# hahnec/stofnet

Hardware: AMD Instinct MI355X
Metric: RF waveforms/sec StofNet inference rf_scale=10 (higher is better)
Workload: dtype f32 via split-fp16 x3 MFMA operands (hi+lo, fp32 accumulate), device-side exact-f32 re-run on fp16 range overflow; 1 GPU; C2 StofNet.forward [4096,1,2000] -> [4096,1,20000] per GPU, upsample_factor=10, SemiGlobalBlock on, seeded-random weights (seed 3008); rows_per_gpu=4096, L=2000, upsample_factor=10, precision=auto

## Files before the change

stofnet_amd/build.py:

```python
from __future__ import annotations

import os
import shutil
import subprocess
import sys

HERE = os.path.dirname(os.path.abspath(__file__))
CSRC = os.path.join(HERE, 'csrc')
LIB = os.path.join(HERE, 'libstofnet_amd.so')
SOURCES = ['pack_weights.cpp', 'convstack.hip', 'shuffle_picker.hip', 'hilbert.hip', 'gradpeak.hip', 'gradpeak_f64.hip', 'neighbors.hip', 'train.hip', 'zonzini.hip', 'sincnet.hip', 'riders.hip']
ARCH = 'gfx950'
EXTRA_FLAGS = {'convstack.hip': ['-fno-slp-vectorize']}


def _hipcc() -> str:
    for cand in (os.environ.get('HIPCC'), shutil.which('hipcc'), '/opt/rocm/bin/hipcc'):
        if cand and os.path.exists(cand):
            return cand
    raise RuntimeError('hipcc not found: the HIP extension cannot be built')


def needs_build() -> bool:
    if not os.path.exists(LIB):
        return True
    t = os.path.getmtime(LIB)
    deps = [os.path.join(CSRC, f) for f in os.listdir(CSRC) if f.endswith(('.hip', '.cpp', '.h'))] + [os.path.join(HERE, '..', 'include', 'stofnet_amd.h')]
    return any(os.path.getmtime(d) > t for d in deps)


def build(force: bool = False, verbose: bool = True) -> str:
    if not force and not needs_build():
        return LIB
    hipcc = _hipcc()
    objdir = os.path.join(HERE, 'build')
    os.makedirs(objdir, exist_ok=True)
    objs = []
    procs = []
    for src in SOURCES:
        path = os.path.join(CSRC, src)
        if not os.path.exists(path):
            raise RuntimeError(f'listed source {path} is missing: refusing to link a library without its symbols')
        obj = os.path.join(objdir, os.path.splitext(src)[0] + '.o')
        cmd = [hipcc, '-O3', '-std=c++17', '-fPIC', '-fconstexpr-steps=100000000', f'--offload-arch={ARCH}', '-x', 'hip'] + \
              EXTRA_FLAGS.get(src, []) + ['-c', path, '-o', obj]
        if verbose:
            print(' '.join(cmd), flush=True)
        procs.append((src, subprocess.Popen(cmd, stdout=subprocess.PIPE, stderr=subprocess.STDOUT, text=True)))
        objs.append(obj)
    for src, pr in procs:
        out, _ = pr.communicate()
        if pr.returncode != 0:
            raise RuntimeError(f'hipcc failed on {src}:\n{out}')
        if verbose and out.strip():
            print(out)
    cmd = [hipcc, '-shared', '-fPIC', f'--offload-arch={ARCH}', '-o', LIB] + objs
    if verbose:
        print(' '.join(cmd), flush=True)
    subprocess.run(cmd, check=True)
    return LIB


if __name__ == '__main__':
    build(force='--force' in sys.argv)
    print(LIB)
```

stofnet_amd/csrc/convstack.hip:

```cpp
#include <hip/hip_runtime.h>
#include <stdlib.h>
#include <type_traits>
#include "stof_common.h"
#include "stof_hip_util.h"

namespace stof {
int launch_conv_cl(const float* x, const float* w, const float* bias, const float* residual, const float* saved, float* y,
                   int64_t N, int64_t L, int32_t cin, int32_t cout, int32_t K, int32_t act, int32_t precision,
                   int32_t period, int32_t valid_len, hipStream_t stream, const int* run_if);
}

using namespace stof;

typedef float floatx16 __attribute__((ext_vector_type(16)));
typedef _Float16 half8 __attribute__((ext_vector_type(8)));
typedef _Float16 half4 __attribute__((ext_vector_type(4)));

namespace {

constexpr int LAG_LAST = 34;
constexpr int SGB_NW = 2;
constexpr int SGB_WAVES_PER_SIMD = (SGB_NW <= 2) ? 2 : 1;
constexpr int ROWB = ROWF * 4;

typedef float float2v __attribute__((ext_vector_type(2)));
typedef float floatx4 __attribute__((ext_vector_type(4)));
typedef _Float16 half2v __attribute__((ext_vector_type(2)));

__device__ __forceinline__ int layer_lag(int j) { return j <= 11 ? 3 * j : LAG_LAST; }

__device__ __forceinline__ float4 ld4(const float* p) { return *reinterpret_cast<const float4*>(p); }
__device__ __forceinline__ void st4(float* p, float4 v) { *reinterpret_cast<float4*>(p) = v; }
__device__ __forceinline__ uint4 ldq(const char* p) { return *reinterpret_cast<const uint4*>(p); }

__device__ __forceinline__ float4 as_f4(uint4 v) {
    return make_float4(__uint_as_float(v.x), __uint_as_float(v.y), __uint_as_float(v.z), __uint_as_float(v.w));
}
__device__ __forceinline__ half8 as_h8(uint4 v) {
    union { uint4 u; half8 h; } c;
    c.u = v;
    return c.h;
}

__device__ __forceinline__ floatx16 mma_fp32(uint4 a, uint4 b, floatx16 c) {
    const float4 af = as_f4(a), bf = as_f4(b);
    c = __builtin_amdgcn_mfma_f32_32x32x2f32(af.x, bf.x, c, 0, 0, 0);
    c = __builtin_amdgcn_mfma_f32_32x32x2f32(af.y, bf.y, c, 0, 0, 0);
    c = __builtin_amdgcn_mfma_f32_32x32x2f32(af.z, bf.z, c, 0, 0, 0);
    c = __builtin_amdgcn_mfma_f32_32x32x2f32(af.w, bf.w, c, 0, 0, 0);
    return c;
}

__device__ __forceinline__ int act_frag_off(int frag, int hh, int lh) { return (32 * hh + 8 * frag + 4 * lh) * 4; }

template <int PREC>
__device__ __forceinline__ void store_act4(char* row, int c0, float4 v) {
    if constexpr (PREC == STOF_PREC_FP32) {
        *reinterpret_cast<float4*>(row + 4 * c0) = v;
    } else {
        half4 hi, lo;
        hi[0] = (_Float16)v.x; hi[1] = (_Float16)v.y; hi[2] = (_Float16)v.z; hi[3] = (_Float16)v.w;
        lo[0] = (_Float16)(v.x - (float)hi[0]); lo[1] = (_Float16)(v.y - (float)hi[1]);
        lo[2] = (_Float16)(v.z - (float)hi[2]); lo[3] = (_Float16)(v.w - (float)hi[3]);
        *reinterpret_cast<half4*>(row + 2 * c0) = hi;
        *reinterpret_cast<half4*>(row + 128 + 2 * c0) = lo;
    }
}

__device__ __forceinline__ float opaque_one() {
    float one;
    asm volatile("s_mov_b32 %0, 1.0" : "=s"(one));
    return one;
}
__device__ __forceinline__ float mix_add(_Float16 h, float v, float one) { return __builtin_fmaf((float)h, one, v); }
__device__ __forceinline__ float mix_sub(_Float16 h, float v, float one) { return __builtin_fmaf(-(float)h, one, v); }
__device__ __forceinline__ half2v cvt_h2(float a, float b) {
    const float2v v = {a, b};
    return __builtin_convertvector(v, half2v);
}
__device__ __forceinline__ unsigned h2_bits(half2v h) {
    union { half2v h; unsigned u; } c;
    c.h = h;
    return c.u;
}
__device__ __forceinline__ half2v bits_h2(unsigned u) {
    union { half2v h; unsigned u; } c;
    c.u = u;
    return c.h;
}
// ... 800 lines not shown
                    for (int gg = 0; gg < 4; ++gg) epi_store(NT - 1, gg, o[gg]);
                };
                if (inplace) tail(std::true_type{});
                else tail(std::false_type{});
                STAMP_ADD(5);
                __syncthreads();
                STAMP_ADD(2);
                continue;
            }
            auto last_chunks = [&]() {
#pragma unroll
                for (int cc = 0; cc < BODY_CHUNKS_LAST; cc += 2) { do_chunk(wf[0], bf0, bf1, cc); do_chunk(wf[1], bf1, bf0, cc + 1); }
            };
            last_chunks();
            STAMP_ADD(4);

            {
                bool valid[NT];
                int tt[NT], nn[NT];
#pragma unroll
                for (int k = 0; k < NT; ++k) {
                    const int off = 32 * (NT * ni + k) + ln;
                    const int g = R0 + off;
                    decode_row(nR, tR, off, nn[k], tt[k]);
                    int nw, tw;
                    vmap(n0 + nn[k], tt[k], nw, tw);
                    valid[k] = (g >= 0) && (g < gend) && (tt[k] < L) && (tw >= 0) && (tw < Ltrue) &&
                               (tt[k] >= p.halo) && (tt[k] < p.halo + p.seg_len);
                    nn[k] = nw - n0;
                    tt[k] = tw;
                }
                if (p.status != nullptr) {
                    bool bad = false;
#pragma unroll
                    for (int k = 0; k < NT; ++k)
#pragma unroll
                        for (int e = 0; e < 16; ++e) bad = bad || !(fabsf(acc[k][e]) <= 3.0e38f);
                    if (__any(bad) && lane == 0) atomicOr(p.status, 1);
                }
#pragma unroll
                for (int k = 0; k < NT; ++k) {
                    if (!valid[k]) continue;
                    float* const orow = p.y + ((size_t)(n0 + nn[k]) * Ltrue + tt[k]) * r;
#pragma unroll
                    for (int gg = 0; gg < 4; ++gg) {
                        const int c0 = 32 * mi + 8 * gg + 4 * lh;
                        if (c0 >= r) continue;
                        const float vv[4] = {acc[k][4 * gg], acc[k][4 * gg + 1], acc[k][4 * gg + 2], acc[k][4 * gg + 3]};
                        if ((r & 3) == 0) {
                            st4(orow + c0, make_float4(vv[0], vv[1], vv[2], vv[3]));
                        } else {
#pragma unroll
                            for (int e = 0; e < 4; ++e)
                                if (c0 + e < r) orow[c0 + e] = vv[e];
                        }
                    }
                }
            }
            STAMP_ADD(5);
            __syncthreads();
            STAMP_ADD(2);
            }
        }
    }
#ifdef STOF_STAMPS
    if (lane == 0 && p.stamps) {
        unsigned long long* o = p.stamps + ((size_t)blockIdx.x * 4 + wave) * 8;
        for (int i = 0; i < 6; ++i) o[i] = tsum[i];
        o[6] = stamp() - tstart;
        o[7] = (unsigned long long)nsteps;
    }
#endif
}

constexpr int BODY_P2_C1F = 640;
#include "body_p2.h"

struct SgbParams {
    const float* x;
    float* pooled;
    const float* c1;
    const float* cbias;
    const float* chunks;
    int N, L, P, tiles_per_wf;
    const int* run_if;
    unsigned char* arg;
};

template <int PREC, int NW, bool ARG = false>
__global__ __launch_bounds__(256, SGB_WAVES_PER_SIMD) void sgb_contract_pool_kernel(const SgbParams p) {
    constexpr int SHAPE = PREC == STOF_PREC_F16X3 ? 16 : 32;
    static_assert(!ARG || PREC == STOF_PREC_F16X3, "the arg-max output lives in the split-fp16 form");
    static_assert(NW % 2 == 0, "80*NW must be a multiple of 32");
    constexpr int ROWS = SGB_SCALE * NW;
    constexpr int MT = ROWS / 32;
    constexpr int TR = ROWS + 4;
    constexpr int RAWN = TR + 8;
    constexpr int RF = SHAPE == 16 ? ROWF16 : ROWF;
    constexpr int ROWB = RF * 4;
    extern __shared__ __attribute__((aligned(16))) float smem[];
    char* const act = reinterpret_cast<char*>(smem);
    float* const raw = smem + TR * RF;

    const int tid = threadIdx.x;
    const int lane = tid & 63, wave = tid >> 6;
    const int ln = lane & 31, lh = lane >> 5;
    const int n = blockIdx.x / p.tiles_per_wf;
    const int w0 = (blockIdx.x - n * p.tiles_per_wf) * NW;
    const int L = p.L;
    const int tbase = SGB_SCALE * w0 - 2;
    if (p.run_if != nullptr && *p.run_if == 0) return;

    const uint4* const wbase = reinterpret_cast<const uint4*>(p.chunks) + wave * 64 + lane;
    auto wload = [&](int c, int f) -> uint4 { return wbase[((size_t)c * FRAGS_PER_CHUNK + f) * 256]; };
    uint4 wf[2][FRAGS_PER_CHUNK];
#pragma unroll
    for (int f = 0; f < FRAGS_PER_CHUNK; ++f) {
        wf[0][f] = wload(0, f);
        wf[1][f] = wload(1, f);
    }

    for (int i = tid; i < RAWN; i += 256) {
        const int t = tbase - 4 + i;
        raw[i] = (t >= 0 && t < L) ? p.x[(size_t)n * L + t] : 0.f;
    }
    __syncthreads();
    {
        const int cq = tid & 15, rl = tid >> 4;
        float w1[4][9], b1[4];
#pragma unroll
        for (int i = 0; i < 4; ++i) {
#pragma unroll
            for (int d = 0; d < 9; ++d) w1[i][d] = p.c1[(4 * cq + i) * 10 + d];
            b1[i] = p.c1[(4 * cq + i) * 10 + 9];
        }
        for (int row = rl; row < TR; row += 16) {
            const int t = tbase + row;
            float v[4];
#pragma unroll
            for (int i = 0; i < 4; ++i) {
                float a = b1[i];
#pragma unroll
                for (int d = 0; d < 9; ++d) a = fmaf(w1[i][d], raw[row + d], a);
                v[i] = fmaxf(a, 0.f);
            }
            const bool valid = (t >= 0) && (t < L);
            store_act4<PREC>(act + row * ROWB, 4 * cq,
                             valid ? make_float4(v[0], v[1], v[2], v[3]) : make_float4(0.f, 0.f, 0.f, 0.f));
        }
    }
    __syncthreads();

    int c = 0;
    if constexpr (SHAPE == 16) {
        constexpr int MW = SGB_SCALE / 16;
        const int j16 = lane & 15, q4 = lane >> 4;
        for (int ocb = 0; ocb < 4; ++ocb) {
            floatx4 acc[NW][MW][2];
#pragma unroll
            for (int w = 0; w < NW; ++w)
#pragma unroll
                for (int m = 0; m < MW; ++m)
#pragma unroll
                    for (int nt = 0; nt < 2; ++nt)
#pragma unroll
                        for (int e = 0; e < 4; ++e) acc[w][m][nt][e] = 0.f;
            constexpr int NUNIT = 10 * NW;
            auto aload = [&](uint4 (&a)[MW][2], int uu) {
                const int cc = uu / NW, w = uu % NW;
                const int d = cc >> 1, hh = cc & 1;
                const char* arow = act + (SGB_SCALE * w + j16 + d) * ROWB + 64 * hh + 16 * q4;
#pragma unroll
                for (int m = 0; m < MW; ++m) {
                    a[m][0] = ldq(arow + 16 * m * ROWB);
                    a[m][1] = ldq(arow + 16 * m * ROWB + 128);
                }
            };
            auto mfma16 = [](const uint4& a, const uint4& b, floatx4 cacc) {
                return __builtin_amdgcn_mfma_f32_16x16x32_f16(as_h8(a), as_h8(b), cacc, 0, 0, 0);
            };
            auto do_unit = [&](uint4 (&acur)[MW][2], uint4 (&anext)[MW][2], int uu) {
                const int cc = uu / NW, w = uu % NW;
                uint4 (&wq)[FRAGS_PER_CHUNK] = wf[cc & 1];
                const int c2 = (c + 2 < SGB_NCHUNK) ? c + 2 : 0;
                aload(anext, uu + 1 < NUNIT ? uu + 1 : 0);
#pragma unroll
                for (int m = 0; m < MW; ++m) {
                    acc[w][m][0] = mfma16(acur[m][0], wq[0], acc[w][m][0]);
                    acc[w][m][1] = mfma16(acur[m][0], wq[2], acc[w][m][1]);
                    acc[w][m][0] = mfma16(acur[m][1], wq[0], acc[w][m][0]);
                    acc[w][m][1] = mfma16(acur[m][1], wq[2], acc[w][m][1]);
                    acc[w][m][0] = mfma16(acur[m][0], wq[1], acc[w][m][0]);
                    acc[w][m][1] = mfma16(acur[m][0], wq[3], acc[w][m][1]);
                }
                if (w == NW - 1) {
#pragma unroll
                    for (int f = 0; f < FRAGS_PER_CHUNK; ++f) wq[f] = wload(c2, f);
                    ++c;
                }
#pragma unroll
                for (int i = 0; i < MW * 2; ++i) {
                    __builtin_amdgcn_sched_group_barrier(0x008, 3, 0);
                    __builtin_amdgcn_sched_group_barrier(0x100, 1, 0);
                }
                if (w == NW - 1) __builtin_amdgcn_sched_group_barrier(0x020, FRAGS_PER_CHUNK, 0);
                __builtin_amdgcn_sched_barrier(0);
            };
            uint4 af0[MW][2], af1[MW][2];
            if (ocb == 0) aload(af0, 0);
            static_assert(NUNIT % 2 == 0, "units alternate between two fragment sets");
#pragma unroll
            for (int uu = 0; uu < NUNIT; uu += 2) {
                do_unit(af0, af1, uu);
                do_unit(af1, af0, uu + 1);
            }
#pragma unroll
            for (int nt = 0; nt < 2; ++nt) {
                const int oc = 128 * ocb + 32 * wave + 16 * nt + j16;
                const float bias = p.cbias[oc];
#pragma unroll
                for (int w = 0; w < NW; ++w) {
                    float mval = -INFINITY;
                    if constexpr (ARG) {
                        int bi = 0;
#pragma unroll
                        for (int m = 0; m < MW; ++m)
#pragma unroll
                            for (int e = 0; e < 4; ++e) {
                                const float v = acc[w][m][nt][e];
                                const bool up = v > mval;
                                mval = up ? v : mval;
                                bi = up ? 16 * m + 4 * q4 + e : bi;
                            }
#pragma unroll
                        for (int off = 16; off <= 32; off <<= 1) {
                            const float ov = __shfl_xor(mval, off);
                            const int oi = __shfl_xor(bi, off);
                            const bool take = (ov > mval) || (ov == mval && oi < bi);
                            mval = take ? ov : mval;
                            bi = take ? oi : bi;
                        }
                        if (q4 == 0 && w0 + w < p.P) p.arg[((size_t)n * p.P + w0 + w) * NF_SGB + oc] = (unsigned char)bi;
                    } else {
#pragma unroll
                        for (int m = 0; m < MW; ++m)
#pragma unroll
                            for (int e = 0; e < 4; ++e) mval = fmaxf(mval, acc[w][m][nt][e]);
                        mval = fmaxf(mval, __shfl_xor(mval, 16));
                        mval = fmaxf(mval, __shfl_xor(mval, 32));
                    }
                    mval += bias;
                    mval = mval > 0.f ? mval : 0.01f * mval;
                    if (q4 == 0 && w0 + w < p.P)
                        p.pooled[((size_t)n * p.P + w0 + w) * NF_SGB + oc] = mval;
                }
            }
        }
    } else {
    for (int ocb = 0; ocb < 4; ++ocb) {
        floatx16 acc[MT];
#pragma unroll
        for (int m = 0; m < MT; ++m)
#pragma unroll
            for (int e = 0; e < 16; ++e) acc[m][e] = 0.f;

        constexpr int UPC = FRAGS_PER_CHUNK;
        constexpr int NUNIT = 10 * UPC;
        auto aload = [&](uint4 (&a)[MT], int uu) {
            const int cc = uu / UPC, sub = uu % UPC;
            const int d = cc >> 1, hh = cc & 1;
            const char* arow = act + (ln + d) * ROWB;
#pragma unroll
            for (int m = 0; m < MT; ++m) a[m] = ldq(arow + 32 * m * ROWB + act_frag_off(sub, hh, lh));
        };
        auto do_unit = [&](uint4 (&acur)[MT], uint4 (&anext)[MT], int uu) {
            const int cc = uu / UPC, sub = uu % UPC;
            uint4 (&w)[FRAGS_PER_CHUNK] = wf[cc & 1];
            const int c2 = (c + 2 < SGB_NCHUNK) ? c + 2 : 0;
            aload(anext, uu + 1 < NUNIT ? uu + 1 : 0);
#pragma unroll
            for (int m = 0; m < MT; ++m) acc[m] = mma_fp32(acur[m], w[sub], acc[m]);
            w[sub] = wload(c2, sub);
#pragma unroll
            for (int i = 0; i < MT; ++i) {
                __builtin_amdgcn_sched_group_barrier(0x008, 4, 0);
                __builtin_amdgcn_sched_group_barrier(0x100, 1, 0);
            }
            if (sub == UPC - 1) ++c;
            __builtin_amdgcn_sched_barrier(0);
        };
        uint4 af0[MT], af1[MT];
        if (ocb == 0) aload(af0, 0);
#pragma unroll
        for (int uu = 0; uu < NUNIT; uu += 2) {
            do_unit(af0, af1, uu);
            do_unit(af1, af0, uu + 1);
        }
        const int oc = 128 * ocb + 32 * wave + ln;
        const float bias = p.cbias[oc];
        float wmax[NW];
#pragma unroll
        for (int w = 0; w < NW; ++w) wmax[w] = -INFINITY;
#pragma unroll
        for (int m = 0; m < MT; ++m)
#pragma unroll
            for (int v = 0; v < 16; ++v) {
                const int w = (32 * m + 8 * (v >> 2)) / SGB_SCALE;
                wmax[w] = fmaxf(wmax[w], acc[m][v]);
            }
#pragma unroll
        for (int w = 0; w < NW; ++w) {
            float mval = fmaxf(wmax[w], __shfl_xor(wmax[w], 32));
            mval += bias;
            mval = mval > 0.f ? mval : 0.01f * mval;
            if (lh == 0 && w0 + w < p.P)
                p.pooled[((size_t)n * p.P + w0 + w) * NF_SGB + oc] = mval;
        }
    }
    }
}

__global__ __launch_bounds__(256) void onsets_finalize_kernel(const OnsetPartial* __restrict__ ws, int nslots, int nb, int r,
                                                              int half, int* __restrict__ counts, int* __restrict__ idx,
                                                              long long idx_cap) {
    const int lane = threadIdx.x & 63;
    const int row = blockIdx.x * 4 + (threadIdx.x >> 6);
    if (row >= nb) return;
    const OnsetPartial* e = ws + (size_t)row * nslots;
    float m = -INFINITY, lo = INFINITY;
    for (int s = lane; s < nslots; s += 64)
        if (e[s].written) { m = fmaxf(m, e[s].m); lo = fminf(lo, e[s].lo); }
#pragma unroll
    for (int o = 32; o > 0; o >>= 1) { m = fmaxf(m, __shfl_xor(m, o)); lo = fminf(lo, __shfl_xor(lo, o)); }
    const bool emit = (m > 0.f) || (m < 0.f && (lo == m || half == 0));
    int nout = 0;
    if (emit) {
        const unsigned long long lt_mask = (lane == 0) ? 0ull : (~0ull >> (64 - lane));
        int* out = idx + (long long)row * idx_cap;
        for (int s0 = 0; s0 < nslots; s0 += 64) {
            const int sl = s0 + lane;
            unsigned long long match = __ballot(sl < nslots && e[sl].written && e[sl].m == m);
            while (match) {
            const int s = s0 + __builtin_ctzll(match);
            match &= match - 1;
            const OnsetPartial p = e[s];
            for (int q0 = 0; q0 < 16 * r; q0 += 64) {
                const int q = q0 + lane, j = q / r, c = q - j * r;
                const bool hit = q < 16 * r && ((p.eq[c & 3] >> (j + 16 * (c >> 2))) & 1ull);
                const unsigned long long hm = __ballot(hit);
                if (hit) {
                    const long long pos = nout + __builtin_popcountll(hm & lt_mask);
                    if (pos < idx_cap) out[pos] = (p.tw_base + j) * r + c;
                }
                nout += __builtin_popcountll(hm);
            }
            }
        }
    }
    if (lane == 0) counts[row] = nout;
}

constexpr int BODY_S = 192, BODY_RING = 256, BODY_RAWRING = 256;
inline bool body_p2_rows_ok(int seg_len, int halo) { return seg_len + 2 * halo + GAP >= 2 * BODY_S; }
constexpr int ONSET_MAX_SEGS = 32;

constexpr int64_t onset_seg_slots(int64_t seg_len) { return seg_len / 16 + 2; }
constexpr int64_t onset_max_slots(int64_t L) { return L / 16 + 3 * ONSET_MAX_SEGS; }

struct OnsetArgs {
    OnsetPartial* ws;
    int32_t* counts;
    int32_t* idx;
    int64_t idx_cap;
    int half;
};
constexpr int64_t SUB_BATCH = 4096;

constexpr size_t sgb_lds_bytes(int rowf) {
    return (size_t)((SGB_SCALE * SGB_NW + 4) * rowf + SGB_SCALE * SGB_NW + 12) * sizeof(float);
}

template <int PREC>
int launch_forward(const stof_net_desc* desc, const void* packed_dev, const float* x, float* y, int64_t N,
                   int64_t L, void* workspace, hipStream_t stream, void* const* events, int32_t* status,
                   const int32_t* run_if, const OnsetArgs* onsets = nullptr) {
    const int force_nseg_log2 = desc->seg_policy > 0 ? desc->seg_policy - 1 : -1;
    const int r = desc->upsample_factor;
    const bool has_sgb = desc->semi_global_scale != 1;
    const int64_t P = L / SGB_SCALE;
    const int64_t rem = L - P * SGB_SCALE;

    const float* base = static_cast<const float*>(packed_dev);
    uint64_t off = sizeof(PackedHeader) / sizeof(float);
    const float* c1 = base + off;      off += 64 * 10;
    const float* bias = base + off;    off += 13 * 64;
    const float* body = base + off;    off += (uint64_t)BODY_NCHUNK * BODY_CHUNK_F;
    const float* last16 = nullptr;
    if (PREC == STOF_PREC_F16X3 && r <= 16) { last16 = base + off; off += LAST16_F; }
    const float* cbias = base + off;   off += NF_SGB;
    const float* cchunks = base + off; off += (uint64_t)SGB_NCHUNK * SGB_CHUNK_F;
    const float* ew = base + off;      off += 5ull * NF_SGB * NF;
    const float* ebias = base + off;

    static const bool body_p2 = PREC == STOF_PREC_F16X3 && body_p2_enabled();
    constexpr int RF = PREC == STOF_PREC_F16X3 ? ROWF16 : ROWF;
    using Lds = BodyLds<BODY_S, BODY_RING, BODY_RAWRING, RF>;
    const size_t body_p2_bytes = Lds::BYTES + BODY_P2_C1F * sizeof(float);
    const auto body_kernel = &body_sweep_kernel<PREC, BODY_S, BODY_RING, BODY_RAWRING>;
    const auto body_p2_kernel = &body_sweep_p2_kernel<BODY_S, BODY_RING, BODY_RAWRING>;
    const auto sgb_kernel = &sgb_contract_pool_kernel<PREC, SGB_NW>;
    const size_t sgb_bytes = sgb_lds_bytes(RF);
    static LdsLimitOnce body_lds, body_p2_lds, sgb_lds;
    if (int st = body_lds.ensure(reinterpret_cast<const void*>(body_kernel), (int)Lds::BYTES)) return st;
    if (body_p2)
        if (int st = body_p2_lds.ensure(reinterpret_cast<const void*>(body_p2_kernel), (int)body_p2_bytes)) return st;
    if (int st = sgb_lds.ensure(reinterpret_cast<const void*>(sgb_kernel), (int)sgb_bytes)) return st;
    const int ncu = device_cu_count();

    for (int64_t b0 = 0; b0 < N; b0 += SUB_BATCH) {
        const int64_t nb = (N - b0) < SUB_BATCH ? (N - b0) : SUB_BATCH;
        const float* xb = x + b0 * L;
        float* yb = y ? y + b0 * L * r : nullptr;
        float* pooled = nullptr;
        float* sgb = nullptr;
        const bool ev = events && b0 == 0;
        if (ev) (void)hipEventRecord(static_cast<hipEvent_t>(events[0]), stream);
        if (has_sgb && P > 0) {
            pooled = static_cast<float*>(workspace);
            sgb = pooled + nb * P * NF_SGB;
            SgbParams sp;
            sp.x = xb; sp.pooled = pooled; sp.c1 = c1; sp.cbias = cbias; sp.chunks = cchunks;
            sp.N = (int)nb; sp.L = (int)L; sp.P = (int)P;
            sp.tiles_per_wf = (int)((P + SGB_NW - 1) / SGB_NW);
            sp.run_if = run_if;
            sp.arg = nullptr;
            hipLaunchKernelGGL(sgb_kernel, dim3((unsigned)(nb * sp.tiles_per_wf)), dim3(256), sgb_bytes, stream, sp);
            if (ev) (void)hipEventRecord(static_cast<hipEvent_t>(events[1]), stream);
            {
                const int st = stof::launch_conv_cl(pooled, ew, ebias, nullptr, nullptr, sgb, 1, nb * (P + 2), NF_SGB, NF, 5,
                                                     2, PREC, (int)(P + 2), (int)P, stream, run_if);
                if (st != STOF_OK) return st;
            }
            if (ev) (void)hipEventRecord(static_cast<hipEvent_t>(events[2]), stream);
        } else if (ev) {
            (void)hipEventRecord(static_cast<hipEvent_t>(events[1]), stream);
            (void)hipEventRecord(static_cast<hipEvent_t>(events[2]), stream);
        }
        BodyParams bp;
        bp.x = xb; bp.sgb = (has_sgb && P > 0) ? sgb : nullptr; bp.y = yb;
        bp.c1 = c1; bp.bias = bias; bp.chunks = body; bp.last16 = last16;
        bp.N = (int)nb; bp.L = (int)L; bp.r = r; bp.P = (int)P; bp.rem_half = (int)(rem / 2);
        bp.stamps = nullptr;
        bp.dump = nullptr; bp.dump_stride = 0;
        bp.gin = nullptr; bp.fwd_dump = nullptr;
        bp.status = status;
        bp.run_if = run_if;
        bp.nseg_log2 = 0;
        {
            int64_t best = -1;
            for (int k = 0; k <= 5; ++k) {
                const int64_t ns = (int64_t)1 << k;
                if (k > 0 && L / ns < BODY_S / 2) break;
                const int64_t lv = (L + ns - 1) / ns + (k > 0 ? 76 : 0);
                const int64_t nvk = nb * ns;
                const int64_t w = nvk < ncu ? nvk : ncu;
                const int64_t per = (nvk + w - 1) / w;
                const int64_t steps = (per * (lv + GAP) - GAP + LAG_LAST + BODY_S - 1) / BODY_S;
                if (best < 0 || steps < best) { best = steps; bp.nseg_log2 = k; }
            }
        }
        int64_t nseg = (int64_t)1 << bp.nseg_log2;
        if (force_nseg_log2 >= 0) { bp.nseg_log2 = force_nseg_log2; nseg = (int64_t)1 << force_nseg_log2; }
        bp.seg_len = (int)((L + nseg - 1) / nseg);
        bp.halo = nseg > 1 ? 38 : 0;
        const int64_t nv = nb * nseg;
        bp.N = (int)nv;
        bp.onset_ws = nullptr; bp.onset_slots = 0; bp.onset_seg_slots = 0;
        if (onsets != nullptr) {
            bp.onset_seg_slots = (int)onset_seg_slots(bp.seg_len);
            bp.onset_slots = (int)(nseg * bp.onset_seg_slots);
            bp.onset_ws = onsets->ws;
            if (hipMemsetAsync(onsets->ws, 0, (size_t)nb * bp.onset_slots * sizeof(OnsetPartial), stream) != hipSuccess)
                return STOF_ERR_HIP;
        }
#ifdef STOF_STAMPS
        if (workspace) bp.stamps = reinterpret_cast<unsigned long long*>(static_cast<char*>(workspace) + (size_t)(nb * P * (NF_SGB + NF)) * sizeof(float) + 256);
#endif
        int64_t wgs = nv < ncu ? nv : ncu;
        bp.wf_per_wg = (int)((nv + wgs - 1) / wgs);
        wgs = (nv + bp.wf_per_wg - 1) / bp.wf_per_wg;
        if (body_p2 && body_p2_rows_ok(bp.seg_len, bp.halo))
            hipLaunchKernelGGL(body_p2_kernel, dim3((unsigned)wgs), dim3(256), body_p2_bytes, stream, bp);
        else
            hipLaunchKernelGGL(body_kernel, dim3((unsigned)wgs), dim3(256), Lds::BYTES, stream, bp);
        if (ev) (void)hipEventRecord(static_cast<hipEvent_t>(events[3]), stream);
        if (onsets != nullptr)
            hipLaunchKernelGGL(onsets_finalize_kernel, dim3((unsigned)((nb + 3) / 4)), dim3(256), 0, stream, onsets->ws,
                               bp.onset_slots, (int)nb, r, onsets->half, onsets->counts + b0, onsets->idx + b0 * onsets->idx_cap,
                               (long long)onsets->idx_cap);
    }
    if (hipGetLastError() != hipSuccess) return STOF_ERR_HIP;
    return STOF_OK;
}

int forward_impl(const stof_net_desc* desc, const void* packed_dev, const float* x, float* y, int64_t N, int64_t L,
                 void* workspace, size_t workspace_bytes, void* stream_, void* const* events, int32_t* status,
                 const int32_t* run_if = nullptr, const OnsetArgs* onsets = nullptr) {
    if (!desc || N < 0 || L < 0) return STOF_ERR_BAD_ARG;
    if (desc->precision != STOF_PREC_FP32 && desc->precision != STOF_PREC_F16X3) return STOF_ERR_UNSUPPORTED;
    if (desc->seg_policy < 0 || desc->seg_policy > 6) return STOF_ERR_UNSUPPORTED;
    const int r = desc->upsample_factor;
    if (r < 1 || r > 64) return STOF_ERR_UNSUPPORTED;
    const bool has_sgb = desc->semi_global_scale != 1;
    if (has_sgb && desc->semi_global_scale != SGB_SCALE) return STOF_ERR_UNSUPPORTED;
    const int64_t P = L / SGB_SCALE;
    if (has_sgb && L > 0 && P == 0) return STOF_ERR_POOL_EMPTY;
    if (has_sgb && ((L - P * SGB_SCALE) & 1)) return STOF_ERR_ODD_SGB_REMAINDER;
    if (N == 0 || L == 0) return STOF_OK;
    if (!packed_dev || !x || (!y && !onsets)) return STOF_ERR_BAD_ARG;
    if ((L + GAP) * SUB_BATCH > 0x7fffffffLL) return STOF_ERR_UNSUPPORTED;
    if (has_sgb && (!workspace || workspace_bytes < stof_forward_workspace_bytes(desc, N, L)))
        return STOF_ERR_WORKSPACE;
    hipStream_t stream = static_cast<hipStream_t>(stream_);
// ... 230 lines not shown
    bp.x = x; bp.sgb = has_sgb ? sgb_expand : nullptr; bp.y = y;
    bp.c1 = base; bp.bias = base + 640; bp.chunks = base + 640 + 13 * 64;
    bp.last16 = r <= 16 ? bp.chunks + (size_t)BODY_NCHUNK * BODY_CHUNK_F : nullptr;
    bp.L = (int)L; bp.r = r; bp.P = (int)P; bp.rem_half = (int)((L - P * SGB_SCALE) / 2);
    bp.stamps = nullptr; bp.status = nullptr; bp.run_if = nullptr;
    bp.onset_ws = nullptr; bp.onset_slots = 0; bp.onset_seg_slots = 0;
    bp.dump = dump; bp.dump_stride = (long long)N * L * NF;
    bp.gin = nullptr; bp.fwd_dump = nullptr;
#ifdef STOF_STAMPS
    bp.stamps = train_stamp_buf(0);
#endif
    int64_t wgs = 0;
    if (int st = train_sweep_geometry(desc, bp, N, L, &wgs)) return st;
    if (p2 && !body_p2_rows_ok(bp.seg_len, bp.halo)) {
        if (split) return STOF_ERR_UNSUPPORTED;
        auto k3 = &body_sweep_kernel<STOF_PREC_F16X3, BODY_S, BODY_RING, BODY_RAWRING, true, false>;
        static LdsLimitOnce lds3;
        if (int st = lds3.ensure(reinterpret_cast<const void*>(k3), (int)Lds16::BYTES)) return st;
        hipLaunchKernelGGL(k3, dim3((unsigned)wgs), dim3(256), Lds16::BYTES, stream, bp);
        return hipGetLastError() == hipSuccess ? STOF_OK : STOF_ERR_HIP;
    }
    hipLaunchKernelGGL(kernel, dim3((unsigned)wgs), dim3(256), lds_bytes, stream, bp);
    return hipGetLastError() == hipSuccess ? STOF_OK : STOF_ERR_HIP;
}

extern "C" int stof_train_sweep(const stof_net_desc* desc, const void* blob_dev, const float* x, const float* sgb_expand,
                                float* dump, float* y, int64_t N, int64_t L, void* stream) {
    return train_sweep_impl(desc, blob_dev, x, sgb_expand, dump, y, N, L, stream, false);
}
extern "C" int stof_train_sweep_split(const stof_net_desc* desc, const void* blob_dev, const float* x, const float* sgb_expand,
                                      float* dump, float* y, int64_t N, int64_t L, void* stream) {
    return train_sweep_impl(desc, blob_dev, x, sgb_expand, dump, y, N, L, stream, true);
}

namespace {
struct SgbPackArgs {
    const float* c1w; const float* c1b; const float* cw; const float* cb;
    float* blob;
};
__global__ __launch_bounds__(256) void sgb_pack_kernel(const SgbPackArgs a) {
    const long long i = blockIdx.x * 256ll + threadIdx.x;
    const long long n_c1 = 640, n_cb = NF_SGB, n_body = (long long)SGB_NCHUNK * SGB_CHUNK_F * 2;
    if (i < n_c1) {
        const int c = (int)(i / 10), t = (int)(i % 10);
        a.blob[i] = t < 9 ? a.c1w[c * 9 + t] : a.c1b[c];
        return;
    }
    long long k = i - n_c1;
    if (k < n_cb) { a.blob[n_c1 + k] = a.cb[k]; return; }
    k -= n_cb;
    if (k >= n_body) return;
    const int e = (int)(k & 7), lane = (int)((k >> 3) & 63), tile = (int)((k >> 9) & 3), frag = (int)((k >> 11) & 3);
    const int c = (int)(k >> 13);
    const int hh = c & 1, tap = (c >> 1) % 5, ocb = c / 10;
    const int nt = frag >> 1, part = frag & 1, j = lane & 15, q = lane >> 4;
    const int o = 128 * ocb + 32 * tile + 16 * nt + j;
    const float v = a.cw[((size_t)o * NF + 32 * hh + 8 * q + e) * 5 + tap];
    const _Float16 hi = (_Float16)v;
    reinterpret_cast<_Float16*>(a.blob + n_c1 + n_cb)[k] = part == 0 ? hi : (_Float16)(v - (float)hi);
}
}

extern "C" size_t stof_train_sgb_blob_bytes(void) { return (640 + NF_SGB + (size_t)SGB_NCHUNK * SGB_CHUNK_F) * sizeof(float); }

extern "C" int stof_train_sgb_contract_pool(const float* conv1_w, const float* conv1_b, const float* contract_w, const float* contract_b,
                                            void* blob_dev, const float* x, float* pooled, uint8_t* arg, int64_t N, int64_t L,
                                            void* stream_) {
    if (N < 0 || L < 0) return STOF_ERR_BAD_ARG;
    const int64_t P = L / SGB_SCALE;
    if (L > 0 && P == 0) return STOF_ERR_POOL_EMPTY;
    if (N == 0 || L == 0) return STOF_OK;
    if (!conv1_w || !conv1_b || !contract_w || !contract_b || !blob_dev || !x || !pooled || !arg) return STOF_ERR_BAD_ARG;
    hipStream_t stream = static_cast<hipStream_t>(stream_);
    SgbPackArgs a;
    a.c1w = conv1_w; a.c1b = conv1_b; a.cw = contract_w; a.cb = contract_b; a.blob = static_cast<float*>(blob_dev);
    const long long total = 640 + NF_SGB + (long long)SGB_NCHUNK * SGB_CHUNK_F * 2;
    hipLaunchKernelGGL(sgb_pack_kernel, dim3((unsigned)((total + 255) / 256)), dim3(256), 0, stream, a);
    auto kernel = &sgb_contract_pool_kernel<STOF_PREC_F16X3, SGB_NW, true>;
    static LdsLimitOnce lds;
    if (int st = lds.ensure(reinterpret_cast<const void*>(kernel), (int)sgb_lds_bytes(ROWF16))) return st;
    SgbParams sp;
    sp.x = x; sp.pooled = pooled; sp.c1 = a.blob; sp.cbias = a.blob + 640; sp.chunks = a.blob + 640 + NF_SGB;
    sp.N = (int)N; sp.L = (int)L; sp.P = (int)P;
    sp.tiles_per_wf = (int)((P + SGB_NW - 1) / SGB_NW);
    sp.run_if = nullptr; sp.arg = arg;
    if (N * sp.tiles_per_wf > 0x7fffffffLL) return STOF_ERR_UNSUPPORTED;
    hipLaunchKernelGGL(kernel, dim3((unsigned)(N * sp.tiles_per_wf)), dim3(256), sgb_lds_bytes(ROWF16), stream, sp);
    return hipGetLastError() == hipSuccess ? STOF_OK : STOF_ERR_HIP;
}

namespace {
struct SweepPackBwdArgs {
    const float* w[11];
    float* blob;
};
__global__ __launch_bounds__(256) void sweep_pack_bwd_kernel(const SweepPackBwdArgs a) {
    const long long i = blockIdx.x * 256ll + threadIdx.x;
    const long long n_head = 640 + 13 * 64, n_body = (long long)BODY_NCHUNK * BODY_CHUNK_F * 2;
    if (i < n_head) { a.blob[i] = 0.f; return; }
    const long long k = i - n_head;
    if (k >= n_body) return;
    _Float16* const body = reinterpret_cast<_Float16*>(a.blob + n_head);
    const int e = (int)(k & 7), lane = (int)((k >> 3) & 63), blk = (int)((k >> 9) & 1), frag = (int)((k >> 10) & 3);
    const int c = (int)(k >> 12);
    if (c >= 11 * BODY_CHUNKS_K7) { body[k] = (_Float16)0.f; return; }
    const int j = 1 + c / BODY_CHUNKS_K7, cc = c % BODY_CHUNKS_K7;
    const int tap = cc >> 1, hh = cc & 1, m = frag >> 1, part = frag & 1, i16 = lane & 15, q = lane >> 4;
    const int arow = body16_out_channel(blk, m, i16);
    const int b = 32 * hh + 8 * q + e;
    const float v = a.w[11 - j][((size_t)b * NF + arow) * 7 + (6 - tap)];
    const _Float16 hi = (_Float16)v;
    body[k] = part == 0 ? hi : (_Float16)(v - (float)hi);
}
}

extern "C" int stof_train_sweep_bwd_pack(const float* const* conv_weights_dev, void* blob_dev, void* stream) {
    if (!conv_weights_dev || !blob_dev) return STOF_ERR_BAD_ARG;
    SweepPackBwdArgs a;
    for (int i = 0; i < 11; ++i) {
        if (!conv_weights_dev[i]) return STOF_ERR_BAD_ARG;
        a.w[i] = conv_weights_dev[i];
    }
    a.blob = static_cast<float*>(blob_dev);
    const long long total = 640 + 13 * 64 + (long long)BODY_NCHUNK * BODY_CHUNK_F * 2;
    hipLaunchKernelGGL(sweep_pack_bwd_kernel, dim3((unsigned)((total + 255) / 256)), dim3(256), 0, static_cast<hipStream_t>(stream), a);
    return hipGetLastError() == hipSuccess ? STOF_OK : STOF_ERR_HIP;
}

static int train_sweep_bwd_impl(const stof_net_desc* desc, const void* blob_dev, const float* g6, const float* fwd_dump,
                                float* dump, int64_t N, int64_t L, void* stream_, bool split) {
    if (!desc || N < 0 || L < 0) return STOF_ERR_BAD_ARG;
    if (N == 0 || L == 0) return STOF_OK;
    if (!blob_dev || !g6 || !fwd_dump || !dump) return STOF_ERR_BAD_ARG;
    if ((L + GAP) * N > 0x7fffffffLL || N * L * NF > 0x7fffffffffLL) return STOF_ERR_UNSUPPORTED;
    hipStream_t stream = static_cast<hipStream_t>(stream_);
    using Lds16 = BodyLds<BODY_S, BODY_RING, BODY_RAWRING, ROWF16>;
    static const bool p2 = body_p2_enabled();
    if (split && !p2) return STOF_ERR_UNSUPPORTED;
    auto kernel = split ? &body_sweep_p2_kernel<BODY_S, BODY_RING, BODY_RAWRING, true, true, true>
                  : p2  ? &body_sweep_p2_kernel<BODY_S, BODY_RING, BODY_RAWRING, true, true>
                        : &body_sweep_kernel<STOF_PREC_F16X3, BODY_S, BODY_RING, BODY_RAWRING, true, true>;
    const size_t lds_bytes = Lds16::BYTES + (p2 ? BODY_P2_C1F * sizeof(float) : 0);
    static LdsLimitOnce lds[2];
    if (int st = lds[split ? 1 : 0].ensure(reinterpret_cast<const void*>(kernel), (int)lds_bytes)) return st;
    const float* base = static_cast<const float*>(blob_dev);
    BodyParams bp;
    bp.x = nullptr; bp.sgb = nullptr; bp.y = nullptr;
    bp.c1 = base; bp.bias = base + 640; bp.chunks = base + 640 + 13 * 64; bp.last16 = nullptr;
    bp.L = (int)L; bp.r = 1; bp.P = 0; bp.rem_half = 0;
    bp.stamps = nullptr; bp.status = nullptr; bp.run_if = nullptr;
    bp.onset_ws = nullptr; bp.onset_slots = 0; bp.onset_seg_slots = 0;
    bp.dump = dump; bp.dump_stride = (long long)N * L * NF;
    bp.gin = g6; bp.fwd_dump = fwd_dump;
#ifdef STOF_STAMPS
    bp.stamps = train_stamp_buf(1);
#endif
    int64_t wgs = 0;
    if (int st = train_sweep_geometry(desc, bp, N, L, &wgs)) return st;
    if (p2 && !body_p2_rows_ok(bp.seg_len, bp.halo)) {
        if (split) return STOF_ERR_UNSUPPORTED;
        auto k3 = &body_sweep_kernel<STOF_PREC_F16X3, BODY_S, BODY_RING, BODY_RAWRING, true, true>;
        static LdsLimitOnce lds3;
        if (int st = lds3.ensure(reinterpret_cast<const void*>(k3), (int)Lds16::BYTES)) return st;
        hipLaunchKernelGGL(k3, dim3((unsigned)wgs), dim3(256), Lds16::BYTES, stream, bp);
        return hipGetLastError() == hipSuccess ? STOF_OK : STOF_ERR_HIP;
    }
    hipLaunchKernelGGL(kernel, dim3((unsigned)wgs), dim3(256), lds_bytes, stream, bp);
    return hipGetLastError() == hipSuccess ? STOF_OK : STOF_ERR_HIP;
}

// ... 32 lines not shown
```

Baseline: 238,400 waveforms/s.

## Add dedicated MFMA expand kernel for SGB and flatten pooling tile indexing

Adds a dedicated split-fp16 MFMA kernel for the SemiGlobalBlock expand conv (512->64, K=5). It stages pooled activations and weights in LDS per 64-channel block and prefetches the next block into registers. This replaces the generic launch_conv_cl path for the f16x3 precision. It also changes the SGB contract/pool kernel so each block takes NW consecutive global windows across rows instead of tiles per waveform, which removes partially empty tail blocks when P is not a multiple of NW. Both windows of a block now get separate padded LDS regions, which adds a little LDS and index arithmetic.

```diff
diff --git a/stofnet_amd/build.py b/stofnet_amd/build.py
--- a/stofnet_amd/build.py
+++ b/stofnet_amd/build.py
@@ -8,7 +8,7 @@
 HERE = os.path.dirname(os.path.abspath(__file__))
 CSRC = os.path.join(HERE, 'csrc')
 LIB = os.path.join(HERE, 'libstofnet_amd.so')
-SOURCES = ['pack_weights.cpp', 'convstack.hip', 'shuffle_picker.hip', 'hilbert.hip', 'gradpeak.hip', 'gradpeak_f64.hip', 'neighbors.hip', 'train.hip', 'zonzini.hip', 'sincnet.hip', 'riders.hip']
+SOURCES = ['pack_weights.cpp', 'convstack.hip', 'sgb_expand.hip', 'shuffle_picker.hip', 'hilbert.hip', 'gradpeak.hip', 'gradpeak_f64.hip', 'neighbors.hip', 'train.hip', 'zonzini.hip', 'sincnet.hip', 'riders.hip']
 ARCH = 'gfx950'
 EXTRA_FLAGS = {'convstack.hip': ['-fno-slp-vectorize']}
 
diff --git a/stofnet_amd/csrc/convstack.hip b/stofnet_amd/csrc/convstack.hip
--- a/stofnet_amd/csrc/convstack.hip
+++ b/stofnet_amd/csrc/convstack.hip
@@ -5,6 +5,8 @@
 #include "stof_hip_util.h"
 
 namespace stof {
+int launch_sgb_expand(const float* pooled, const float* w, const float* bias, float* sgb, int64_t nb, int64_t P,
+                      hipStream_t stream, const int* run_if);
 int launch_conv_cl(const float* x, const float* w, const float* bias, const float* residual, const float* saved, float* y,
                    int64_t N, int64_t L, int32_t cin, int32_t cout, int32_t K, int32_t act, int32_t precision,
                    int32_t period, int32_t valid_len, hipStream_t stream, const int* run_if);
@@ -971,7 +973,7 @@
     const float* c1;
     const float* cbias;
     const float* chunks;
-    int N, L, P, tiles_per_wf;
+    int N, L, P;
     const int* run_if;
     unsigned char* arg;
 };
@@ -983,8 +985,10 @@
     static_assert(NW % 2 == 0, "80*NW must be a multiple of 32");
     constexpr int ROWS = SGB_SCALE * NW;
     constexpr int MT = ROWS / 32;
-    constexpr int TR = ROWS + 4;
-    constexpr int RAWN = TR + 8;
+    constexpr int WR = SGB_SCALE + 4;
+    constexpr int WRAW = WR + 8;
+    constexpr int TR = NW * WR;
+    constexpr int RAWN = NW * WRAW;
     constexpr int RF = SHAPE == 16 ? ROWF16 : ROWF;
     constexpr int ROWB = RF * 4;
     extern __shared__ __attribute__((aligned(16))) float smem[];
@@ -994,11 +998,16 @@
     const int tid = threadIdx.x;
     const int lane = tid & 63, wave = tid >> 6;
     const int ln = lane & 31, lh = lane >> 5;
-    const int n = blockIdx.x / p.tiles_per_wf;
-    const int w0 = (blockIdx.x - n * p.tiles_per_wf) * NW;
     const int L = p.L;
-    const int tbase = SGB_SCALE * w0 - 2;
+    const int g0 = blockIdx.x * NW;
+    const int gtot = p.N * p.P;
     if (p.run_if != nullptr && *p.run_if == 0) return;
+    auto window = [&](int wi, int& n, int& tbase) -> bool {
+        const int g = g0 + wi;
+        n = g / p.P;
+        tbase = SGB_SCALE * (g - n * p.P) - 2;
+        return g < gtot;
+    };
 
     const uint4* const wbase = reinterpret_cast<const uint4*>(p.chunks) + wave * 64 + lane;
     auto wload = [&](int c, int f) -> uint4 { return wbase[((size_t)c * FRAGS_PER_CHUNK + f) * 256]; };
@@ -1010,8 +1019,11 @@
     }
 
     for (int i = tid; i < RAWN; i += 256) {
-        const int t = tbase - 4 + i;
-        raw[i] = (t >= 0 && t < L) ? p.x[(size_t)n * L + t] : 0.f;
+        const int wi = i / WRAW;
+        int n, tbase;
+        const bool present = window(wi, n, tbase);
+        const int t = tbase - 4 + (i - wi * WRAW);
+        raw[i] = (present && t >= 0 && t < L) ? p.x[(size_t)n * L + t] : 0.f;
     }
     __syncthreads();
     {
@@ -1024,16 +1036,20 @@
             b1[i] = p.c1[(4 * cq + i) * 10 + 9];
         }
         for (int row = rl; row < TR; row += 16) {
-            const int t = tbase + row;
+            const int wi = row / WR;
+            int n, tbase;
+            const bool present = window(wi, n, tbase);
+            const int t = tbase + (row - wi * WR);
+            const float* const rw = raw + row + 8 * wi;
             float v[4];
 #pragma unroll
             for (int i = 0; i < 4; ++i) {
                 float a = b1[i];
 #pragma unroll
-                for (int d = 0; d < 9; ++d) a = fmaf(w1[i][d], raw[row + d], a);
+                for (int d = 0; d < 9; ++d) a = fmaf(w1[i][d], rw[d], a);
                 v[i] = fmaxf(a, 0.f);
             }
-            const bool valid = (t >= 0) && (t < L);
+            const bool valid = present && (t >= 0) && (t < L);
             store_act4<PREC>(act + row * ROWB, 4 * cq,
                              valid ? make_float4(v[0], v[1], v[2], v[3]) : make_float4(0.f, 0.f, 0.f, 0.f));
         }
@@ -1058,7 +1074,7 @@
             auto aload = [&](uint4 (&a)[MW][2], int uu) {
                 const int cc = uu / NW, w = uu % NW;
                 const int d = cc >> 1, hh = cc & 1;
-                const char* arow = act + (SGB_SCALE * w + j16 + d) * ROWB + 64 * hh + 16 * q4;
+                const char* arow = act + (WR * w + j16 + d) * ROWB + 64 * hh + 16 * q4;
 #pragma unroll
                 for (int m = 0; m < MW; ++m) {
                     a[m][0] = ldq(arow + 16 * m * ROWB);
@@ -1129,7 +1145,7 @@
                             mval = take ? ov : mval;
                             bi = take ? oi : bi;
                         }
-                        if (q4 == 0 && w0 + w < p.P) p.arg[((size_t)n * p.P + w0 + w) * NF_SGB + oc] = (unsigned char)bi;
+                        if (q4 == 0 && g0 + w < gtot) p.arg[(size_t)(g0 + w) * NF_SGB + oc] = (unsigned char)bi;
                     } else {
 #pragma unroll
                         for (int m = 0; m < MW; ++m)
@@ -1140,12 +1156,18 @@
                     }
                     mval += bias;
                     mval = mval > 0.f ? mval : 0.01f * mval;
-                    if (q4 == 0 && w0 + w < p.P)
-                        p.pooled[((size_t)n * p.P + w0 + w) * NF_SGB + oc] = mval;
+                    if (q4 == 0 && g0 + w < gtot)
+                        p.pooled[(size_t)(g0 + w) * NF_SGB + oc] = mval;
                 }
             }
         }
     } else {
+    int arow_off[MT];
+#pragma unroll
+    for (int m = 0; m < MT; ++m) {
+        const int r = 32 * m + ln;
+        arow_off[m] = (r + 4 * (r / SGB_SCALE)) * ROWB;
+    }
     for (int ocb = 0; ocb < 4; ++ocb) {
         floatx16 acc[MT];
 #pragma unroll
@@ -1158,9 +1180,9 @@
         auto aload = [&](uint4 (&a)[MT], int uu) {
             const int cc = uu / UPC, sub = uu % UPC;
             const int d = cc >> 1, hh = cc & 1;
-            const char* arow = act + (ln + d) * ROWB;
-#pragma unroll
-            for (int m = 0; m < MT; ++m) a[m] = ldq(arow + 32 * m * ROWB + act_frag_off(sub, hh, lh));
+            const char* arow = act + d * ROWB + act_frag_off(sub, hh, lh);
+#pragma unroll
+            for (int m = 0; m < MT; ++m) a[m] = ldq(arow + arow_off[m]);
         };
         auto do_unit = [&](uint4 (&acur)[MT], uint4 (&anext)[MT], int uu) {
             const int cc = uu / UPC, sub = uu % UPC;
@@ -1202,8 +1224,8 @@
             float mval = fmaxf(wmax[w], __shfl_xor(wmax[w], 32));
             mval += bias;
             mval = mval > 0.f ? mval : 0.01f * mval;
-            if (lh == 0 && w0 + w < p.P)
-                p.pooled[((size_t)n * p.P + w0 + w) * NF_SGB + oc] = mval;
+            if (lh == 0 && g0 + w < gtot)
+                p.pooled[(size_t)(g0 + w) * NF_SGB + oc] = mval;
         }
     }
     }
@@ -1266,7 +1288,7 @@
 constexpr int64_t SUB_BATCH = 4096;
 
 constexpr size_t sgb_lds_bytes(int rowf) {
-    return (size_t)((SGB_SCALE * SGB_NW + 4) * rowf + SGB_SCALE * SGB_NW + 12) * sizeof(float);
+    return (size_t)SGB_NW * ((SGB_SCALE + 4) * rowf + SGB_SCALE + 12) * sizeof(float);
 }
 
 template <int PREC>
@@ -1320,14 +1342,17 @@
             SgbParams sp;
             sp.x = xb; sp.pooled = pooled; sp.c1 = c1; sp.cbias = cbias; sp.chunks = cchunks;
             sp.N = (int)nb; sp.L = (int)L; sp.P = (int)P;
-            sp.tiles_per_wf = (int)((P + SGB_NW - 1) / SGB_NW);
             sp.run_if = run_if;
             sp.arg = nullptr;
-            hipLaunchKernelGGL(sgb_kernel, dim3((unsigned)(nb * sp.tiles_per_wf)), dim3(256), sgb_bytes, stream, sp);
+            hipLaunchKernelGGL(sgb_kernel, dim3((unsigned)((nb * P + SGB_NW - 1) / SGB_NW)), dim3(256), sgb_bytes, stream, sp);
             if (ev) (void)hipEventRecord(static_cast<hipEvent_t>(events[1]), stream);
             {
-                const int st = stof::launch_conv_cl(pooled, ew, ebias, nullptr, nullptr, sgb, 1, nb * (P + 2), NF_SGB, NF, 5,
-                                                     2, PREC, (int)(P + 2), (int)P, stream, run_if);
+                int st;
+                if constexpr (PREC == STOF_PREC_F16X3)
+                    st = stof::launch_sgb_expand(pooled, ew, ebias, sgb, nb, P, stream, run_if);
+                else
+                    st = stof::launch_conv_cl(pooled, ew, ebias, nullptr, nullptr, sgb, 1, nb * (P + 2), NF_SGB, NF, 5,
+                                               2, PREC, (int)(P + 2), (int)P, stream, run_if);
                 if (st != STOF_OK) return st;
             }
             if (ev) (void)hipEventRecord(static_cast<hipEvent_t>(events[2]), stream);
@@ -1724,10 +1749,9 @@
     SgbParams sp;
     sp.x = x; sp.pooled = pooled; sp.c1 = a.blob; sp.cbias = a.blob + 640; sp.chunks = a.blob + 640 + NF_SGB;
     sp.N = (int)N; sp.L = (int)L; sp.P = (int)P;
-    sp.tiles_per_wf = (int)((P + SGB_NW - 1) / SGB_NW);
     sp.run_if = nullptr; sp.arg = arg;
-    if (N * sp.tiles_per_wf > 0x7fffffffLL) return STOF_ERR_UNSUPPORTED;
-    hipLaunchKernelGGL(kernel, dim3((unsigned)(N * sp.tiles_per_wf)), dim3(256), sgb_lds_bytes(ROWF16), stream, sp);
+    if (N * P + SGB_NW > 0x7fffffffLL) return STOF_ERR_UNSUPPORTED;
+    hipLaunchKernelGGL(kernel, dim3((unsigned)((N * P + SGB_NW - 1) / SGB_NW)), dim3(256), sgb_lds_bytes(ROWF16), stream, sp);
     return hipGetLastError() == hipSuccess ? STOF_OK : STOF_ERR_HIP;
 }
 
diff --git a/stofnet_amd/csrc/sgb_expand.hip b/stofnet_amd/csrc/sgb_expand.hip
--- /dev/null
+++ b/stofnet_amd/csrc/sgb_expand.hip
@@ -0,0 +1,191 @@
+#include <hip/hip_runtime.h>
+#include <stdint.h>
+#include "stof_common.h"
+#include "stof_hip_util.h"
+
+typedef float floatx16 __attribute__((ext_vector_type(16)));
+typedef _Float16 half8 __attribute__((ext_vector_type(8)));
+typedef _Float16 half4v __attribute__((ext_vector_type(4)));
+typedef float float4v __attribute__((ext_vector_type(4)));
+
+namespace {
+
+constexpr int EX_ROWS = 256;
+constexpr int EX_K = 5, EX_PAD = 2;
+constexpr int EX_XR = EX_ROWS + EX_K - 1;
+constexpr int EX_CIN = 512, EX_COUT = 64, EX_NCB = EX_CIN / 64;
+constexpr int EX_RF = 68;
+constexpr int EX_RB = EX_RF * 4;
+constexpr int EX_NXR = (EX_XR * 16 + 255) / 256;
+constexpr int EX_NWR = EX_K * EX_COUT * 16 / 256;
+constexpr size_t EX_LDS_BYTES = (size_t)(EX_XR + EX_K * EX_COUT) * EX_RB;
+
+struct ExpandParams {
+    const float* pooled;
+    const float* w;
+    const float* bias;
+    float* sgb;
+    int P, period;
+    int total;
+    const int* run_if;
+};
+
+__device__ __forceinline__ float4 ld4(const float* p) { return *reinterpret_cast<const float4*>(p); }
+__device__ __forceinline__ uint4 ldq(const char* p) { return *reinterpret_cast<const uint4*>(p); }
+
+__device__ __forceinline__ floatx16 mfma_h(uint4 a, uint4 b, floatx16 c) {
+    union U { uint4 u; half8 h; };
+    U x, y;
+    x.u = a; y.u = b;
+    return __builtin_amdgcn_mfma_f32_32x32x16_f16(x.h, y.h, c, 0, 0, 0);
+}
+
+__device__ __forceinline__ void split4(float4 v, uint2& hi, uint2& lo) {
+    const float4v f = {v.x, v.y, v.z, v.w};
+    const half4v h = __builtin_convertvector(f, half4v);
+    const float4v d = f - __builtin_convertvector(h, float4v);
+    const half4v l = __builtin_convertvector(d, half4v);
+    union { half4v h; uint2 u; } a, b;
+    a.h = h; b.h = l;
+    hi = a.u; lo = b.u;
+}
+
+__global__ __launch_bounds__(256) void sgb_expand_kernel(const ExpandParams p) {
+    extern __shared__ __attribute__((aligned(16))) float smem[];
+    char* const xs = reinterpret_cast<char*>(smem);
+    char* const ws = xs + EX_XR * EX_RB;
+    const int tid = threadIdx.x, lane = tid & 63, wave = tid >> 6;
+    const int mi = wave & 1, ni = wave >> 1, ln = lane & 31, lh = lane >> 5;
+    if (p.run_if != nullptr && *p.run_if == 0) return;
+    const int t0 = blockIdx.x * EX_ROWS;
+
+    const int xq = tid & 15;
+    int xsrc[EX_NXR];
+#pragma unroll
+    for (int u = 0; u < EX_NXR; ++u) {
+        const int r = (tid + 256 * u) >> 4;
+        const int t = t0 - EX_PAD + r;
+        int src = -1;
+        if (r < EX_XR && t >= 0 && t < p.total) {
+            const int nn = t / p.period, pp = t - nn * p.period;
+            if (pp < p.P) src = nn * p.P + pp;
+        }
+        xsrc[u] = src;
+    }
+    float4 xreg[EX_NXR], wreg[EX_NWR];
+    auto fetch = [&](int cb) {
+#pragma unroll
+        for (int u = 0; u < EX_NXR; ++u) {
+            float4 v = make_float4(0.f, 0.f, 0.f, 0.f);
+            if (xsrc[u] >= 0) v = ld4(p.pooled + (size_t)xsrc[u] * EX_CIN + 64 * cb + 4 * xq);
+            xreg[u] = v;
+        }
+#pragma unroll
+        for (int u = 0; u < EX_NWR; ++u) {
+            const int i = tid + 256 * u;
+            wreg[u] = ld4(p.w + ((size_t)(i >> 4) * EX_NCB + cb) * 64 + 4 * (i & 15));
+        }
+    };
+    fetch(0);
+
+    floatx16 acc[4], tot[4];
+#pragma unroll
+    for (int j = 0; j < 4; ++j)
+#pragma unroll
+        for (int e = 0; e < 16; ++e) { acc[j][e] = 0.f; tot[j][e] = 0.f; }
+
+    for (int cb = 0; cb < EX_NCB; ++cb) {
+        if (cb > 0) {
+#pragma unroll
+            for (int j = 0; j < 4; ++j)
+#pragma unroll
+                for (int e = 0; e < 16; ++e) { tot[j][e] += acc[j][e]; acc[j][e] = 0.f; }
+            __syncthreads();
+        }
+#pragma unroll
+        for (int u = 0; u < EX_NXR; ++u) {
+            const int r = (tid + 256 * u) >> 4;
+            if (r >= EX_XR) continue;
+            uint2 hi, lo;
+            split4(xreg[u], hi, lo);
+            char* row = xs + r * EX_RB;
+            *reinterpret_cast<uint2*>(row + 8 * xq) = hi;
+            *reinterpret_cast<uint2*>(row + 128 + 8 * xq) = lo;
+        }
+#pragma unroll
+        for (int u = 0; u < EX_NWR; ++u) {
+            const int i = tid + 256 * u;
+            *reinterpret_cast<float4*>(ws + (i >> 4) * EX_RB + 16 * (i & 15)) = wreg[u];
+        }
+        if (cb + 1 < EX_NCB) fetch(cb + 1);
+        __syncthreads();
+
+        const char* const ar0 = ws + (32 * mi + ln) * EX_RB + 16 * lh;
+        const char* const br0 = xs + (128 * ni + ln) * EX_RB + 16 * lh;
+#pragma unroll
+        for (int d = 0; d < EX_K; ++d) {
+#pragma unroll
+            for (int q = 0; q < 4; ++q) {
+                const char* ar = ar0 + d * EX_COUT * EX_RB + 32 * q;
+                const char* br = br0 + d * EX_RB + 32 * q;
+                const uint4 ah = ldq(ar), al = ldq(ar + 128);
+#pragma unroll
+                for (int j = 0; j < 4; ++j) {
+                    const uint4 bh = ldq(br + 32 * j * EX_RB), bl = ldq(br + 32 * j * EX_RB + 128);
+                    acc[j] = mfma_h(ah, bh, acc[j]);
+                    acc[j] = mfma_h(ah, bl, acc[j]);
+                    acc[j] = mfma_h(al, bh, acc[j]);
+                }
+            }
+        }
+    }
+#pragma unroll
+    for (int j = 0; j < 4; ++j)
+#pragma unroll
+        for (int e = 0; e < 16; ++e) acc[j][e] += tot[j][e];
+
+#pragma unroll
+    for (int j = 0; j < 4; ++j) {
+        const int t = t0 + 128 * ni + 32 * j + ln;
+        if (t >= p.total) continue;
+        const int nn = t / p.period, pp = t - nn * p.period;
+        if (pp >= p.P) continue;
+        float* const orow = p.sgb + ((size_t)nn * p.P + pp) * EX_COUT;
+#pragma unroll
+        for (int gg = 0; gg < 4; ++gg) {
+            const int o = 32 * mi + 8 * gg + 4 * lh;
+            const float4 b = ld4(p.bias + o);
+            const float bi[4] = {b.x, b.y, b.z, b.w};
+            float v[4];
+#pragma unroll
+            for (int e = 0; e < 4; ++e) {
+                float x = acc[j][4 * gg + e] + bi[e];
+                x = x > 0.f ? x : 0.01f * x;
+                v[e] = x + 0.f;
+            }
+            *reinterpret_cast<float4*>(orow + o) = make_float4(v[0], v[1], v[2], v[3]);
+        }
+    }
+}
+
+}
+
+namespace stof {
+
+int launch_sgb_expand(const float* pooled, const float* w, const float* bias, float* sgb, int64_t nb, int64_t P,
+                      hipStream_t stream, const int* run_if) {
+    if (nb <= 0 || P <= 0) return STOF_OK;
+    if (!pooled || !w || !bias || !sgb) return STOF_ERR_BAD_ARG;
+    const int64_t total = nb * (P + 2);
+    if (total + EX_ROWS > 0x7fffffffLL) return STOF_ERR_UNSUPPORTED;
+    static LdsLimitOnce lds;
+    if (int st = lds.ensure(reinterpret_cast<const void*>(&sgb_expand_kernel), (int)EX_LDS_BYTES)) return st;
+    ExpandParams p;
+    p.pooled = pooled; p.w = w; p.bias = bias; p.sgb = sgb;
+    p.P = (int)P; p.period = (int)(P + 2); p.total = (int)total;
+    p.run_if = run_if;
+    hipLaunchKernelGGL(sgb_expand_kernel, dim3((unsigned)((total + EX_ROWS - 1) / EX_ROWS)), dim3(256), EX_LDS_BYTES, stream, p);
+    return hipGetLastError() == hipSuccess ? STOF_OK : STOF_ERR_HIP;
+}
+
+}
```

New measurement: 241,700 waveforms/s (median of 6 runs). 1.4% higher.
